# linnanwang/FastGen

Hardware: AMD Instinct MI355X
Metric: images/sec at 4-step distilled (DMD2) sampling (higher is better)
Workload: dtype fp32 (tensors, accumulate) with split-bf16 x3 MFMA conv products; 1 GPU; EDM CIFAR-10 32x32 SongUNet (55.7M params) DMD2 4-step 'sde' sampling, batch=512 per GPU; global_batch=512, sample_steps=4, parallelism=replicas x1 (no data-path collective), graph=True

## Files before the change

### fastgen_amd/csrc/conv_ws3.hip

```cpp
#include "common.h"
#include "conv.h"

namespace {

constexpr int X3_NTHR = 768;
constexpr int X3_KC = 32;
constexpr int X3_PA = 16;
constexpr int X3_PLANE = 3072;
constexpr int X3_ABUF = 8 * X3_PLANE;
constexpr int X3_RING = 4;
constexpr int X3_HOFF = 128 * 512;
constexpr int X3_LDS = X3_HOFF + X3_RING * X3_ABUF;
constexpr int X3_TAPB = 2048;

template <int LOGW>
struct X3Geom {
    static constexpr int W = 1 << LOGW;
    static constexpr int TW = 16, TH = 8;
    static constexpr int IPT = LOGW == 3 ? 2 : 1;
    static constexpr int TCOLS = LOGW == 3 ? 1 : W / TW;
    static constexpr int TPI = LOGW == 3 ? 1 : (W / TH) * TCOLS;
    static constexpr int HW_ = LOGW == 3 ? 2 * W + 3 : TW + 2, HH_ = TH + 2;
    static constexpr int HALO_PIX = HW_ * HH_;
    static constexpr int RS = HW_ * X3_PA;
    static_assert(HALO_PIX * X3_PA <= X3_PLANE && HALO_PIX <= 192, "one halo plane; three producer passes of 64 pixels");
};

__device__ __forceinline__ void x3_barrier() {
    asm volatile("s_waitcnt lgkmcnt(0)\n\ts_barrier" ::: "memory");
}

struct X3Frag {
    bf16x8 hi, lo;
};

template <int RES, int LOGW, int PRO>
__global__ __launch_bounds__(X3_NTHR) void conv3_x3ws_kernel(const ConvArgs a, const int ntiles) {
    using G = X3Geom<LOGW>;
    constexpr bool SUB = RES == RES_SUBPIX;
    constexpr int NTAP = SUB ? 4 : 9;
    constexpr int RN = SUB ? 4 : 3;
    constexpr int NQ = 4 * NTAP;
    constexpr int X3_STEPB = NTAP * X3_TAPB;
    extern __shared__ __attribute__((aligned(16))) char smem[];
    char* const hbuf = smem;
    char* const ring = smem + X3_HOFF;

    const int tid = threadIdx.x;
    const int lane = tid & 63;
    const int wave = __builtin_amdgcn_readfirstlane(tid >> 6);
    const int Cin = a.C1 + a.C2;
    const int nchunk = Cin / X3_KC;
    const int G8 = (int)gridDim.x >> 3;
    const int wg = ((gridDim.x & 7) == 0) ? ((int)blockIdx.x & 7) * G8 + ((int)blockIdx.x >> 3) : (int)blockIdx.x;
    const int gstride = (int)gridDim.x;
    const int my_tiles = (ntiles - wg + gstride - 1) / gstride;
    const int S = my_tiles * nchunk;
    const int NSTEP = S + 3;
    const int H = SUB ? a.Hs : a.H;

    if (wave < 8) {
        const int grp = wave >> 2, wl = wave & 3;
        const int col = lane & 15, g4 = lane >> 4;
        const size_t wstride = (size_t)nchunk * NTAP * 1024;
        const __amdgpu_buffer_rsrc_t wrs = __builtin_amdgcn_make_buffer_rsrc(
            const_cast<__bf16*>(reinterpret_cast<const __bf16*>(a.wpack_ws) + (size_t)(grp * 8 + wl * 2) * wstride), 0, 0x7fffffff,
            0x00020000);
        const int wvoff = lane * 16;
        const int wsb = (int)(wstride * 2);
        const int wphb = SUB ? 16 * wsb : 0;
        int tcur = wg;
        auto load_w = [&](int byte_off) -> X3Frag {
            X3Frag f;
            f.hi = __builtin_bit_cast(bf16x8, __builtin_amdgcn_raw_buffer_load_b128(wrs, wvoff, byte_off, 0));
            f.lo = __builtin_bit_cast(bf16x8, __builtin_amdgcn_raw_buffer_load_b128(wrs, wvoff, byte_off + 1024, 0));
            return f;
        };
        X3Frag wq[RN][2];
#pragma unroll
        for (int j = 0; j < RN; ++j)
#pragma unroll
            for (int nt = 0; nt < 2; ++nt) wq[j][nt] = load_w((tcur & 3) * wphb + nt * wsb + j * X3_TAPB);

        f32x4 acc[8][2];
#pragma unroll
        for (int m = 0; m < 8; ++m)
#pragma unroll
            for (int nt = 0; nt < 2; ++nt) acc[m][nt] = f32x4{0.f, 0.f, 0.f, 0.f};

        const int lane_off = g4 * X3_PLANE + (col + ((G::IPT == 2 && col >= 8) ? 1 : 0)) * X3_PA;
        const int dl0 = col * 512 + ((8 * wl + ((g4) ^ (col & 7))) << 4);
        const int dl1 = col * 512 + ((8 * wl + ((4 + g4) ^ (col & 7))) << 4);

        x3_barrier();
        int c = 0;
        for (int s = 0; s < NSTEP; ++s) {
            const int ls = s - 2 * grp;
            if (ls >= 0 && ls < S) {
                const char* abase = ring + (ls & 3) * X3_ABUF + lane_off + (SUB ? ((tcur >> 1) & 1) * G::RS + (tcur & 1) * X3_PA : 0);
                const int cn = (c + 1 == nchunk) ? 0 : c + 1;
                const int tnext = cn == 0 ? tcur + gstride : tcur;
                const int wcur = (tcur & 3) * wphb + c * X3_STEPB;
                const int wnxt = (ls + 1 < S) ? (tnext & 3) * wphb + cn * X3_STEPB : wcur;
                auto read_x = [&](int q, X3Frag (&xf)[2]) {
                    const int tap = q >> 2, m0 = 2 * (q & 3);
                    const int off = ((SUB ? tap >> 1 : tap / 3) + m0) * G::RS + (SUB ? tap & 1 : tap % 3) * X3_PA;
#pragma unroll
                    for (int m = 0; m < 2; ++m) {
                        xf[m].hi = *reinterpret_cast<const bf16x8*>(abase + off + m * G::RS);
                        xf[m].lo = *reinterpret_cast<const bf16x8*>(abase + off + m * G::RS + 4 * X3_PLANE);
                    }
                };
                auto mma12 = [&](int q, const X3Frag (&xf)[2]) {
                    const int tap = q >> 2, m0 = 2 * (q & 3);
                    const X3Frag(&wf)[2] = wq[tap % RN];
#pragma unroll
                    for (int m = 0; m < 2; ++m)
#pragma unroll
                        for (int nt = 0; nt < 2; ++nt)
                            acc[m0 + m][nt] = __builtin_amdgcn_mfma_f32_16x16x32_bf16(wf[nt].hi, xf[m].lo, acc[m0 + m][nt], 0, 0, 0);
#pragma unroll
                    for (int m = 0; m < 2; ++m)
#pragma unroll
                        for (int nt = 0; nt < 2; ++nt)
                            acc[m0 + m][nt] = __builtin_amdgcn_mfma_f32_16x16x32_bf16(wf[nt].lo, xf[m].hi, acc[m0 + m][nt], 0, 0, 0);
#pragma unroll
                    for (int m = 0; m < 2; ++m)
#pragma unroll
                        for (int nt = 0; nt < 2; ++nt)
                            acc[m0 + m][nt] = __builtin_amdgcn_mfma_f32_16x16x32_bf16(wf[nt].hi, xf[m].hi, acc[m0 + m][nt], 0, 0, 0);
                    if ((q & 3) != 3) return;
                    const int pn = (tap + RN < NTAP) ? wcur + (tap + RN) * X3_TAPB : wnxt + (tap + RN - NTAP) * X3_TAPB;
#pragma unroll
                    for (int nt = 0; nt < 2; ++nt) wq[tap % RN][nt] = load_w(pn + nt * wsb);
                };
                X3Frag x0[2], x1[2];
                read_x(0, x0);
#pragma unroll
                for (int q = 0; q < NQ; q += 2) {
                    read_x(q + 1, x1);
                    __builtin_amdgcn_sched_barrier(0);
                    mma12(q, x0);
                    __builtin_amdgcn_sched_barrier(0);
                    if (q + 2 < NQ) read_x(q + 2, x0);
                    __builtin_amdgcn_sched_barrier(0);
                    mma12(q + 1, x1);
                    __builtin_amdgcn_sched_barrier(0);
                }
                if (c + 1 == nchunk) {
#pragma unroll
                    for (int m = 0; m < 8; ++m) {
                        *reinterpret_cast<f32x4*>(hbuf + m * 8192 + dl0) = acc[m][0];
                        *reinterpret_cast<f32x4*>(hbuf + m * 8192 + dl1) = acc[m][1];
                        acc[m][0] = f32x4{0.f, 0.f, 0.f, 0.f};
                        acc[m][1] = f32x4{0.f, 0.f, 0.f, 0.f};
                    }
                }
                c = cn;
                tcur = tnext;
            }
            x3_barrier();
        }
        return;
    }

    const int ptid = tid - 512;
    const int pw = wave - 8;
    const int oct = ptid & 3;
    const float* src1 = reinterpret_cast<const float*>(a.src1);
    const float* src2 = reinterpret_cast<const float*>(a.src2);
    int hdy[3], hdx[3], hlds[3];
    bool third;
    const int pslot = ptid >> 2;
    const int pimg = (G::IPT == 2 && pslot >= 30) ? 1 : 0;
#pragma unroll
    for (int i = 0; i < 3; ++i) {
        int hy, hx;
        if (G::IPT == 2) {
            const int l = pimg ? min(pslot - 30 + 34 * i, 99) : pslot + 30 * i;
            hy = pimg ? l / 10 : l / 9;
            hx = pimg ? 9 + (l - hy * 10) : l - hy * 9;
            third = pimg ? pslot - 30 + 68 < 100 : true;
        } else {
            const int hq = min(pslot + 64 * i, G::HALO_PIX - 1);
            hy = hq / G::HW_;
            hx = hq - hy * G::HW_;
            third = pslot + 128 < G::HALO_PIX;
        }
        hdy[i] = hy - 1;
        hdx[i] = hx - 1 - pimg * (G::W + 1);
        hlds[i] = oct * X3_PLANE + hy * G::RS + hx * X3_PA;
    }

    auto tile_coord = [&](int t, int& n, int& slot, int& row0, int& col0) {
        if (SUB) t >>= 2;
        n = t * G::IPT / G::TPI;
        slot = t - n * G::TPI / G::IPT;
        row0 = (slot / G::TCOLS) * G::TH;
        col0 = (slot % G::TCOLS) * G::TW;
    };

    struct Staged {
        f32x4 raw[3][2];
        float2 ab[8];
    };
    unsigned off1[3], off2[3];
    bool valid[3];
    const float2* abn = a.ab;
    auto tile_setup = [&](int t) __attribute__((always_inline)) {
        int n, slot, row0, col0;
        tile_coord(t, n, slot, row0, col0);
        bool in_batch = true;
        if (G::IPT == 2) {
            n += pimg;
            in_batch = n < a.B;
            n = min(n, a.B - 1);
        }
#pragma unroll
        for (int i = 0; i < 3; ++i) {
            const int y = row0 + hdy[i], x = col0 + hdx[i];
            valid[i] = (y >= 0) && (y < H) && (x >= 0) && (x < G::W) && (i < 2 || third) && in_batch;
            const int yc = min(max(y, 0), H - 1), xc = min(max(x, 0), G::W - 1);
            const int sy = (RES == RES_UP) ? (yc >> 1) : yc, sx = (RES == RES_UP) ? (xc >> 1) : xc;
            const unsigned pix = (unsigned)((n * a.Hs + sy) * a.Ws + sx);
            off1[i] = (pix * (unsigned)a.C1 + oct * 8) * 4u;
            off2[i] = (pix * (unsigned)a.C2 + oct * 8) * 4u;
        }
        abn = a.ab + (size_t)n * Cin;
    };
    auto stage_load = [&](Staged& st, int t, int c32) __attribute__((always_inline)) {
        if (c32 == 0) tile_setup(t);
        const bool first = c32 * X3_KC < a.C1;
        const char* base = first ? reinterpret_cast<const char*>(src1) + c32 * (X3_KC * 4)
                                 : reinterpret_cast<const char*>(src2) + (c32 * X3_KC - a.C1) * 4;
#pragma unroll
        for (int i = 0; i < 3; ++i) {
            const char* p = base + (first ? off1[i] : off2[i]);
            st.raw[i][0] = *reinterpret_cast<const f32x4*>(p);
            st.raw[i][1] = *reinterpret_cast<const f32x4*>(p + 16);
        }
        if (PRO == PRO_NONE) return;
        const float2* p = abn + c32 * X3_KC + oct * 8;
#pragma unroll
        for (int j = 0; j < 8; j += 2) {
            const f32x4 q = *reinterpret_cast<const f32x4*>(p + j);
            st.ab[j] = make_float2(q[0], q[1]);
            st.ab[j + 1] = make_float2(q[2], q[3]);
        }
    };
    auto stage_store = [&](const Staged& st, char* abuf) __attribute__((always_inline)) {
#pragma unroll
        for (int i = 0; i < 3; ++i) {
            float v[8];
#pragma unroll
            for (int j = 0; j < 8; ++j) {
                v[j] = st.raw[i][j >> 2][j & 3];
                if (PRO != PRO_NONE) v[j] = silu_f<true>(fmaf(v[j], st.ab[j].x, st.ab[j].y));
            }
            bf16x8 hi, lo;
            split8(v, hi, lo);
            typedef __attribute__((ext_vector_type(4))) unsigned u32x4;
            u32x4 wh = __builtin_bit_cast(u32x4, hi), wl_ = __builtin_bit_cast(u32x4, lo);
#pragma unroll
            for (int j = 0; j < 4; ++j) {
                wh[j] = valid[i] ? wh[j] : 0u;
                wl_[j] = valid[i] ? wl_[j] : 0u;
            }
            if (i < 2 || third) {
                *reinterpret_cast<u32x4*>(abuf + hlds[i]) = wh;
                *reinterpret_cast<u32x4*>(abuf + hlds[i] + 4 * X3_PLANE) = wl_;
            }
        }
    };

    const int chq = lane & 31, psub = lane >> 5;
    float* const out = reinterpret_cast<float*>(a.out);
    const float* const resid = reinterpret_cast<const float*>(a.resid);
    const bool has_resid = __builtin_amdgcn_readfirstlane(resid != nullptr);
    auto retire_half = [&](int t, int half) __attribute__((always_inline)) {
        int n, slot, row0, col0;
        tile_coord(t, n, slot, row0, col0);
        const int co = half * 128 + chq * 4;
        const int nimg = G::IPT == 2 ? min(2, a.B - n) : 1;
        f32x4 radd[G::IPT];
#pragma unroll
        for (int k = 0; k < G::IPT; ++k) {
            radd[k] = f32x4{0.f, 0.f, 0.f, 0.f};
            if (a.bias) radd[k] = *reinterpret_cast<const f32x4*>(a.bias + co);
            const int nk = G::IPT == 2 ? min(n + k, a.B - 1) : n;
            if (a.temb) radd[k] += *reinterpret_cast<const f32x4*>(a.temb + (size_t)nk * a.temb_stride + co);
            radd[k] *= a.scale;
        }
        constexpr int OW = SUB ? 2 * G::W : G::W, OST = SUB ? 2 : 1;
        const int ph = t & 3;
        const size_t tb = SUB ? (((size_t)n * (2 * H) + 2 * row0 + (ph >> 1)) * OW + 2 * col0 + (ph & 1)) * 256 + co
                              : (((size_t)n * H + row0) * G::W + col0) * 256 + co;
        const int rs = (SUB || G::IPT == 2) ? 0 : a.rshift;
        const size_t rtb = (SUB || G::IPT == 2) ? tb : (((size_t)n * (H >> rs) + (row0 >> rs)) * (G::W >> rs) + (col0 >> rs)) * 256 + co;
        float ssum[G::IPT] = {}, ssq[G::IPT] = {};
#pragma unroll 1
        for (int grp8 = 0; grp8 < 2; ++grp8) {
            f32x4 rr[8], dv[8];
            unsigned go[8];
#pragma unroll
            for (int j = 0; j < 8; ++j) {
                const int px = pw * 32 + 2 * (grp8 * 8 + j) + psub;
                unsigned rgo;
                if (G::IPT == 2) {
                    go[j] = (unsigned)((((j >> 2) * OW + OST * (px >> 4)) * OW + OST * (px & 7)) * 256);
                    rgo = go[j];
                } else {
                    go[j] = (unsigned)((OST * (px >> 4) * OW + OST * (px & 15)) * 256);
                    rgo = SUB ? go[j] : (unsigned)((((px >> 4) >> rs) * (G::W >> rs) + ((px & 15) >> rs)) * 256);
                }
                rr[j] = f32x4{0.f, 0.f, 0.f, 0.f};
                if (has_resid && (G::IPT == 1 || (j >> 2) < nimg)) rr[j] = *reinterpret_cast<const f32x4*>(resid + rtb + rgo);
                dv[j] = *reinterpret_cast<const f32x4*>(hbuf + px * 512 + ((chq ^ (px & 7)) << 4));
            }
#pragma unroll
            for (int j = 0; j < 8; ++j) {
                const int k = G::IPT == 2 ? j >> 2 : 0;
                if (G::IPT == 2 && k >= nimg) continue;
                f32x4 v;
#pragma unroll
                for (int e = 0; e < 4; ++e) v[e] = fmaf(dv[j][e], a.scale, radd[k][e]);
                if (has_resid) {
#pragma unroll
                    for (int e = 0; e < 4; ++e) v[e] = fmaf(rr[j][e], a.scale, v[e]);
                }
                *reinterpret_cast<f32x4*>(out + tb + go[j]) = v;
                ssum[k] += (v[0] + v[1]) + (v[2] + v[3]);
                ssq[k] += (v[0] * v[0] + v[1] * v[1]) + (v[2] * v[2] + v[3] * v[3]);
            }
        }
#pragma unroll
        for (int k = 0; k < G::IPT; ++k) {
            ssum[k] += __shfl_xor(ssum[k], 32);
            ssq[k] += __shfl_xor(ssq[k], 32);
            const size_t sl = SUB ? ((size_t)(n + k) * G::TPI + slot) * 4 + ph : (size_t)(n + k) * G::TPI + slot;
            if (a.stats && psub == 0 && k < nimg) a.stats[(sl * 4 + pw) * 64 + half * 32 + chq] = make_float2(ssum[k], ssq[k]);
        }
    };

    auto advance = [&](int& t, int& cc) {
        if (++cc == nchunk) {
            cc = 0;
            t += gstride;
        }
    };
    Staged st;
    int t1 = wg, c1 = 0;
    stage_load(st, t1, c1);
    stage_store(st, ring);
    advance(t1, c1);
    x3_barrier();
    int sa = 0;
    for (int s = 0; s < NSTEP; ++s) {
        const bool more = s + 1 < S;
        if (more) stage_load(st, t1, c1);
        if (sa == 0 && s >= nchunk && s <= S) retire_half(wg + (s / nchunk - 1) * gstride, 0);
        if (sa == 2 % nchunk && s - 2 >= nchunk && s - 2 <= S && (s - 2) % nchunk == 0) retire_half(wg + ((s - 2) / nchunk - 1) * gstride, 1);
        if (more) {
            stage_store(st, ring + ((s + 1) & 3) * X3_ABUF);
            advance(t1, c1);
        }
        if (++sa == nchunk) sa = 0;
        x3_barrier();
    }
}

__global__ void pack_conv_weights_x3ws_kernel(const float* __restrict__ w, __bf16* __restrict__ out, int cout, int cin) {
    const size_t total = (size_t)cout * cin * 9;
    const int nstep = cin / X3_KC;
    for (size_t idx = (size_t)blockIdx.x * blockDim.x + threadIdx.x; idx < total; idx += (size_t)gridDim.x * blockDim.x) {
        size_t t = idx;
        const int j = t % 8; t /= 8;
        const int lane = t % 64; t /= 64;
        const int tap = t % 9; t /= 9;
        const int step = t % nstep; t /= nstep;
        const int n16 = (int)t;
        const int co = n16 * 16 + (lane & 15);
        const int ci = step * X3_KC + 8 * (lane >> 4) + j;
        const float v = w[((size_t)co * cin + ci) * 9 + tap];
        const __bf16 hi = (__bf16)v;
        const size_t o = (idx / 512) * 1024 + (idx % 512);
        out[o] = hi;
        out[o + 512] = (__bf16)(v - (float)hi);
    }
}

__global__ void pack_conv_weights_x3sub_kernel(const float* __restrict__ w, __bf16* __restrict__ out, int cout, int cin) {
    const size_t total = (size_t)16 * cout * cin;
    const int nstep = cin / X3_KC, ng = cout / 16;
    for (size_t idx = (size_t)blockIdx.x * blockDim.x + threadIdx.x; idx < total; idx += (size_t)gridDim.x * blockDim.x) {
        size_t t = idx;
        const int j = t % 8; t /= 8;
        const int lane = t % 64; t /= 64;
        const int tap = t % 4; t /= 4;
        const int step = t % nstep; t /= nstep;
        const int n16 = t % ng; t /= ng;
        const int py = (int)t >> 1, px = (int)t & 1, ty = tap >> 1, tx = tap & 1;
        const int co = n16 * 16 + (lane & 15);
        const int ci = step * X3_KC + 8 * (lane >> 4) + j;
        const int ky0 = py ? 2 * ty : ty, ky1 = py ? ty + 1 : 2 * ty;
        const int kx0 = px ? 2 * tx : tx, kx1 = px ? tx + 1 : 2 * tx;
        const float* wp = w + ((size_t)co * cin + ci) * 9;
        float v = 0.f;
        for (int ky = ky0; ky <= ky1; ++ky)
            for (int kx = kx0; kx <= kx1; ++kx) v += wp[ky * 3 + kx];
        const __bf16 hi = (__bf16)v;
        const size_t o = (idx / 512) * 1024 + (idx % 512);
        out[o] = hi;
        out[o + 512] = (__bf16)(v - (float)hi);
    }
}

int g_x3_cus[16] = {};

template <int RES, int LOGW, int PRO>
int launch_x3_one(const ConvArgs& a, hipStream_t stream, bool prepare_only) {
    using G = X3Geom<LOGW>;
    auto kern = conv3_x3ws_kernel<RES, LOGW, PRO>;
    int dev = 0;
    if (hipGetDevice(&dev) != hipSuccess || dev < 0 || dev >= 16) return (int)hipErrorInvalidDevice;
    static bool attr_done[16] = {};
    if (!attr_done[dev]) {
        hipError_t e = hipFuncSetAttribute(reinterpret_cast<const void*>(kern), hipFuncAttributeMaxDynamicSharedMemorySize, X3_LDS);
        if (e != hipSuccess) return (int)e;
        attr_done[dev] = true;
    }
    if (!g_x3_cus[dev]) {
        int n = 0;
        if (hipDeviceGetAttribute(&n, hipDeviceAttributeMultiprocessorCount, dev) != hipSuccess || n <= 0) return (int)hipErrorUnknown;
        g_x3_cus[dev] = n;
    }
    if (prepare_only) return 0;
    const int ntiles = (a.B * G::TPI + G::IPT - 1) / G::IPT * (RES == RES_SUBPIX ? 4 : 1);
    const int grid = ntiles < g_x3_cus[dev] ? ntiles : g_x3_cus[dev];
    hipLaunchKernelGGL(kern, dim3(grid), dim3(X3_NTHR), X3_LDS, stream, a, ntiles);
    return (int)hipGetLastError();
}

}

int conv_x3ws_stat_slots(int W, int res) {
    if (res == RES_SUBPIX) return (W == 32 ? X3Geom<4>::TPI : X3Geom<3>::TPI) * 16;
    return (W == 32 ? X3Geom<5>::TPI : W == 16 ? X3Geom<4>::TPI : X3Geom<3>::TPI) * 4;
}

bool conv_x3ws_shape_ok(int cout, int cin, int res) {
    return cout == 256 && (res == 32 || res == 16 || res == 8) && (cin % X3_KC) == 0 && cin / X3_KC >= 4;
}

bool conv_x3ws_supported(int ks, int pro, int res, int outmode, const ConvArgs& a) {
    const int cin = a.C1 + a.C2;
    const size_t src_bytes = (size_t)a.B * a.Hs * a.Ws * (size_t)(a.C1 > a.C2 ? a.C1 : a.C2) * 4;
    if (src_bytes >= (1ull << 32)) return false;
    if (res == RES_SUBPIX)
        return ks == 3 && outmode == OUT_NHWC && pro == PRO_GN_SILU && a.ab && a.H == a.W && a.Hs == a.Ws && a.H == 2 * a.Hs && (a.Ws == 16 || a.Ws == 8) &&
               conv_x3ws_shape_ok(a.Cout, cin, a.Ws) && (a.C1 % X3_KC) == 0 && a.wpack_ws && !a.rshift;
    if (ks != 3 || outmode != OUT_NHWC || a.H != a.W || !conv_x3ws_shape_ok(a.Cout, cin, a.W) || (a.C1 % X3_KC) || !a.wpack_ws) return false;
    if (a.W == 8 && res != RES_NONE) return false;
    if (a.rshift && (a.rshift != 1 || !a.resid || a.W == 8 || res != RES_NONE)) return false;
    if (pro == PRO_NONE) return res == RES_NONE && a.Hs == a.H && a.Ws == a.W;
    return pro == PRO_GN_SILU && (res == RES_NONE || res == RES_UP) && a.ab != nullptr;
}

int launch_conv_x3ws(int res, const ConvArgs& a, hipStream_t stream, bool prepare_only, int pro) {
    if (res == RES_SUBPIX) {
        if (pro != PRO_GN_SILU || (a.Ws != 16 && a.Ws != 8)) return (int)hipErrorInvalidValue;
        return a.Ws == 16 ? launch_x3_one<RES_SUBPIX, 4, PRO_GN_SILU>(a, stream, prepare_only) : launch_x3_one<RES_SUBPIX, 3, PRO_GN_SILU>(a, stream, prepare_only);
    }
    if (pro == PRO_NONE || a.W == 8) {
        if (res != RES_NONE) return (int)hipErrorInvalidValue;
        if (a.W == 8)
            return pro == PRO_NONE ? launch_x3_one<RES_NONE, 3, PRO_NONE>(a, stream, prepare_only)
                                   : launch_x3_one<RES_NONE, 3, PRO_GN_SILU>(a, stream, prepare_only);
        return a.W == 32 ? launch_x3_one<RES_NONE, 5, PRO_NONE>(a, stream, prepare_only) : launch_x3_one<RES_NONE, 4, PRO_NONE>(a, stream, prepare_only);
    }
    if (a.W == 32)
        return res == RES_UP ? launch_x3_one<RES_UP, 5, PRO_GN_SILU>(a, stream, prepare_only) : launch_x3_one<RES_NONE, 5, PRO_GN_SILU>(a, stream, prepare_only);
    return res == RES_UP ? launch_x3_one<RES_UP, 4, PRO_GN_SILU>(a, stream, prepare_only) : launch_x3_one<RES_NONE, 4, PRO_GN_SILU>(a, stream, prepare_only);
}

int launch_pack_conv_weights_x3ws(const float* w_oihw, void* wpack_ws, int cout, int cin, hipStream_t stream) {
    const size_t total = (size_t)cout * cin * 9;
    const int grid = (int)((total + 255) / 256 < 4096 ? (total + 255) / 256 : 4096);
    hipLaunchKernelGGL(pack_conv_weights_x3ws_kernel, dim3(grid), dim3(256), 0, stream, w_oihw, (__bf16*)wpack_ws, cout, cin);
    return (int)hipGetLastError();
}

int launch_pack_conv_weights_x3sub(const float* w_oihw, void* wpack_sub, int cout, int cin, hipStream_t stream) {
    const size_t total = (size_t)16 * cout * cin;
    const int grid = (int)((total + 255) / 256 < 4096 ? (total + 255) / 256 : 4096);
    hipLaunchKernelGGL(pack_conv_weights_x3sub_kernel, dim3(grid), dim3(256), 0, stream, w_oihw, (__bf16*)wpack_sub, cout, cin);
    return (int)hipGetLastError();
}
```

Before: 2832 img/s.

## Interleave paired 8x8 images in LDS halo and skip zero-padding rows

For the 8x8 resolution where two images share a tile, the halo layout now interleaves the two images column-wise (slot = 2*x + img) with a single shared padding row that wraps. Padding slots are zero-filled once at kernel start instead of being written on every stage. The MFMA loop skips reads and multiplies for rows that are always padding in the non-subpixel case, and the producer needs only two staging passes instead of three. The epilogue assigns one image per lane half, which removes the per-image loops and the cross-lane shuffle. Compile-time checks verify that LDS reads are bank-conflict free and that the slot mapping covers every position, but the change adds considerable indexing complexity.

```diff
diff --git a/fastgen_amd/csrc/conv_ws3.hip b/fastgen_amd/csrc/conv_ws3.hip
--- a/fastgen_amd/csrc/conv_ws3.hip
+++ b/fastgen_amd/csrc/conv_ws3.hip
@@ -20,11 +20,71 @@
     static constexpr int IPT = LOGW == 3 ? 2 : 1;
     static constexpr int TCOLS = LOGW == 3 ? 1 : W / TW;
     static constexpr int TPI = LOGW == 3 ? 1 : (W / TH) * TCOLS;
-    static constexpr int HW_ = LOGW == 3 ? 2 * W + 3 : TW + 2, HH_ = TH + 2;
+    static constexpr int HW_ = IPT == 2 ? 2 * (W + 2) : TW + 2, HH_ = IPT == 2 ? TH + 1 : TH + 2;
     static constexpr int HALO_PIX = HW_ * HH_;
     static constexpr int RS = HW_ * X3_PA;
+    static constexpr int NI = IPT == 2 ? 2 : 3;
+    static constexpr int ZSLOTS = IPT == 2 ? HALO_PIX - 2 * W * W : 0;
     static_assert(HALO_PIX * X3_PA <= X3_PLANE && HALO_PIX <= 192, "one halo plane; three producer passes of 64 pixels");
+
+    static constexpr int prow(int r) { return (IPT == 2 && r == TH + 1) ? 0 : r; }
+    static constexpr int pix_slot(int img, int y, int x) { return prow(y + 1) * HW_ + (IPT == 2 ? 2 * (x + 1) + img : x + 1); }
+    static constexpr int read_slot(int col, int r, int c) { return prow(r) * HW_ + col + IPT * c; }
+    static constexpr int stage_pix(int ps, int i) { return (ps & 31) + 32 * i; }
+    static constexpr int stage_slot(int ps, int i) { return pix_slot(ps >> 5, stage_pix(ps, i) >> 3, stage_pix(ps, i) & 7); }
+    static constexpr int zero_slot(int z) { return z < HW_ ? z : (1 + ((z - HW_) >> 2)) * HW_ + ((z - HW_) & 3) + (((z - HW_) & 2) ? HW_ - 4 : 0); }
+    static constexpr bool is_zero_slot(int s) { return IPT == 2 && (s < HW_ || s % HW_ < 2 || s % HW_ >= HW_ - 2); }
 };
+
+constexpr int x3_b128_group(int lane) {
+    const int l = lane & 31;
+    return 2 * (lane >> 5) + ((l < 4 || (l >= 12 && l < 16) || (l >= 20 && l < 28)) ? 0 : 1);
+}
+template <int LOGW>
+constexpr bool x3_reads_conflict_free() {
+    using G = X3Geom<LOGW>;
+    for (int r = 0; r <= G::TH + 1; ++r)
+        for (int c = 0; c < 3; ++c)
+            for (int grp = 0; grp < 4; ++grp) {
+                unsigned seen = 0;
+                for (int lane = 0; lane < 64; ++lane) {
+                    if (x3_b128_group(lane) != grp) continue;
+                    const int byte = (lane >> 4) * X3_PLANE + G::read_slot(lane & 15, r, c) * X3_PA;
+                    const unsigned bit = 1u << ((byte >> 4) & 15);
+                    if (seen & bit) return false;
+                    seen |= bit;
+                }
+            }
+    return true;
+}
+constexpr bool x3_pair_layout_ok() {
+    using G = X3Geom<3>;
+    for (int col = 0; col < 16; ++col)
+        for (int r = 0; r <= G::TH + 1; ++r)
+            for (int c = 0; c < 3; ++c) {
+                const int img = col & 1, y = r - 1, x = (col >> 1) + c - 1;
+                const int s = G::read_slot(col, r, c);
+                const bool pad = y < 0 || y >= G::W || x < 0 || x >= G::W;
+                if (s != G::pix_slot(img, y, x) || G::is_zero_slot(s) != pad || s < 0 || s >= G::HALO_PIX) return false;
+            }
+    bool used[G::HALO_PIX] = {};
+    for (int ps = 0; ps < 64; ++ps)
+        for (int i = 0; i < G::NI; ++i) {
+            const int p = G::stage_pix(ps, i), s = G::stage_slot(ps, i);
+            if (p < 0 || p >= G::W * G::W || s < 0 || s >= G::HALO_PIX || G::is_zero_slot(s) || used[s]) return false;
+            used[s] = true;
+        }
+    for (int z = 0; z < G::ZSLOTS; ++z) {
+        const int s = G::zero_slot(z);
+        if (s < 0 || s >= G::HALO_PIX || !G::is_zero_slot(s) || used[s]) return false;
+        used[s] = true;
+    }
+    for (int s = 0; s < G::HALO_PIX; ++s)
+        if (!used[s]) return false;
+    return true;
+}
+static_assert(x3_reads_conflict_free<3>() && x3_reads_conflict_free<4>() && x3_reads_conflict_free<5>(), "activation reads: one LDS cycle per lane group");
+static_assert(X3Geom<3>::ZSLOTS == 52 && x3_pair_layout_ok(), "8x8 pair layout: reads, staging and zero fill");
 
 __device__ __forceinline__ void x3_barrier() {
     asm volatile("s_waitcnt lgkmcnt(0)\n\ts_barrier" ::: "memory");
@@ -88,7 +148,7 @@
 #pragma unroll
             for (int nt = 0; nt < 2; ++nt) acc[m][nt] = f32x4{0.f, 0.f, 0.f, 0.f};
 
-        const int lane_off = g4 * X3_PLANE + (col + ((G::IPT == 2 && col >= 8) ? 1 : 0)) * X3_PA;
+        const int lane_off = g4 * X3_PLANE + G::read_slot(col, 0, 0) * X3_PA;
         const int dl0 = col * 512 + ((8 * wl + ((g4) ^ (col & 7))) << 4);
         const int dl1 = col * 512 + ((8 * wl + ((4 + g4) ^ (col & 7))) << 4);
 
@@ -97,18 +157,24 @@
         for (int s = 0; s < NSTEP; ++s) {
             const int ls = s - 2 * grp;
             if (ls >= 0 && ls < S) {
-                const char* abase = ring + (ls & 3) * X3_ABUF + lane_off + (SUB ? ((tcur >> 1) & 1) * G::RS + (tcur & 1) * X3_PA : 0);
+                const int py = SUB ? (tcur >> 1) & 1 : 0, px = SUB ? tcur & 1 : 0;
+                const char* abase = ring + (ls & 3) * X3_ABUF + lane_off + (SUB ? G::read_slot(0, py, px) * X3_PA : 0);
+                const int wrap = (SUB && G::IPT == 2 && py) ? -(G::TH + 1) * G::RS : 0;
                 const int cn = (c + 1 == nchunk) ? 0 : c + 1;
                 const int tnext = cn == 0 ? tcur + gstride : tcur;
                 const int wcur = (tcur & 3) * wphb + c * X3_STEPB;
                 const int wnxt = (ls + 1 < S) ? (tnext & 3) * wphb + cn * X3_STEPB : wcur;
+                auto zero_row = [](int tap, int m) { return !SUB && G::IPT == 2 && (tap / 3 + m == 0 || tap / 3 + m == G::TH + 1); };
                 auto read_x = [&](int q, X3Frag (&xf)[2]) {
                     const int tap = q >> 2, m0 = 2 * (q & 3);
-                    const int off = ((SUB ? tap >> 1 : tap / 3) + m0) * G::RS + (SUB ? tap & 1 : tap % 3) * X3_PA;
+                    const int ty = SUB ? tap >> 1 : tap / 3, tx = SUB ? tap & 1 : tap % 3;
 #pragma unroll
                     for (int m = 0; m < 2; ++m) {
-                        xf[m].hi = *reinterpret_cast<const bf16x8*>(abase + off + m * G::RS);
-                        xf[m].lo = *reinterpret_cast<const bf16x8*>(abase + off + m * G::RS + 4 * X3_PLANE);
+                        if (zero_row(tap, m0 + m)) continue;
+                        const int r = ty + m0 + m;
+                        const int off = G::read_slot(0, r, tx) * X3_PA + ((SUB && G::IPT == 2 && r == G::TH) ? wrap : 0);
+                        xf[m].hi = *reinterpret_cast<const bf16x8*>(abase + off);
+                        xf[m].lo = *reinterpret_cast<const bf16x8*>(abase + off + 4 * X3_PLANE);
                     }
                 };
                 auto mma12 = [&](int q, const X3Frag (&xf)[2]) {
@@ -118,17 +184,20 @@
                     for (int m = 0; m < 2; ++m)
 #pragma unroll
                         for (int nt = 0; nt < 2; ++nt)
-                            acc[m0 + m][nt] = __builtin_amdgcn_mfma_f32_16x16x32_bf16(wf[nt].hi, xf[m].lo, acc[m0 + m][nt], 0, 0, 0);
+                            if (!zero_row(tap, m0 + m))
+                                acc[m0 + m][nt] = __builtin_amdgcn_mfma_f32_16x16x32_bf16(wf[nt].hi, xf[m].lo, acc[m0 + m][nt], 0, 0, 0);
 #pragma unroll
                     for (int m = 0; m < 2; ++m)
 #pragma unroll
                         for (int nt = 0; nt < 2; ++nt)
-                            acc[m0 + m][nt] = __builtin_amdgcn_mfma_f32_16x16x32_bf16(wf[nt].lo, xf[m].hi, acc[m0 + m][nt], 0, 0, 0);
+                            if (!zero_row(tap, m0 + m))
+                                acc[m0 + m][nt] = __builtin_amdgcn_mfma_f32_16x16x32_bf16(wf[nt].lo, xf[m].hi, acc[m0 + m][nt], 0, 0, 0);
 #pragma unroll
                     for (int m = 0; m < 2; ++m)
 #pragma unroll
                         for (int nt = 0; nt < 2; ++nt)
-                            acc[m0 + m][nt] = __builtin_amdgcn_mfma_f32_16x16x32_bf16(wf[nt].hi, xf[m].hi, acc[m0 + m][nt], 0, 0, 0);
+                            if (!zero_row(tap, m0 + m))
+                                acc[m0 + m][nt] = __builtin_amdgcn_mfma_f32_16x16x32_bf16(wf[nt].hi, xf[m].hi, acc[m0 + m][nt], 0, 0, 0);
                     if ((q & 3) != 3) return;
                     const int pn = (tap + RN < NTAP) ? wcur + (tap + RN) * X3_TAPB : wnxt + (tap + RN - NTAP) * X3_TAPB;
 #pragma unroll
@@ -169,27 +238,33 @@
     const int oct = ptid & 3;
     const float* src1 = reinterpret_cast<const float*>(a.src1);
     const float* src2 = reinterpret_cast<const float*>(a.src2);
-    int hdy[3], hdx[3], hlds[3];
-    bool third;
+    constexpr int NI = G::NI;
+    int hdy[NI], hdx[NI], hlds[NI];
+    bool third = true;
     const int pslot = ptid >> 2;
-    const int pimg = (G::IPT == 2 && pslot >= 30) ? 1 : 0;
-#pragma unroll
-    for (int i = 0; i < 3; ++i) {
-        int hy, hx;
+    const int pimg = G::IPT == 2 ? pslot >> 5 : 0;
+#pragma unroll
+    for (int i = 0; i < NI; ++i) {
         if (G::IPT == 2) {
-            const int l = pimg ? min(pslot - 30 + 34 * i, 99) : pslot + 30 * i;
-            hy = pimg ? l / 10 : l / 9;
-            hx = pimg ? 9 + (l - hy * 10) : l - hy * 9;
-            third = pimg ? pslot - 30 + 68 < 100 : true;
+            const int p = G::stage_pix(pslot, i);
+            hdy[i] = p >> 3;
+            hdx[i] = p & 7;
+            hlds[i] = oct * X3_PLANE + G::stage_slot(pslot, i) * X3_PA;
         } else {
             const int hq = min(pslot + 64 * i, G::HALO_PIX - 1);
-            hy = hq / G::HW_;
-            hx = hq - hy * G::HW_;
+            const int hy = hq / G::HW_, hx = hq - hy * G::HW_;
             third = pslot + 128 < G::HALO_PIX;
-        }
-        hdy[i] = hy - 1;
-        hdx[i] = hx - 1 - pimg * (G::W + 1);
-        hlds[i] = oct * X3_PLANE + hy * G::RS + hx * X3_PA;
+            hdy[i] = hy - 1;
+            hdx[i] = hx - 1;
+            hlds[i] = oct * X3_PLANE + hy * G::RS + hx * X3_PA;
+        }
+    }
+    if constexpr (G::IPT == 2) {
+        typedef __attribute__((ext_vector_type(4))) unsigned u32x4;
+        for (int idx = ptid; idx < X3_RING * 8 * G::ZSLOTS; idx += 256) {
+            const int plane = idx / G::ZSLOTS;
+            *reinterpret_cast<u32x4*>(ring + plane * X3_PLANE + G::zero_slot(idx - plane * G::ZSLOTS) * X3_PA) = u32x4{0u, 0u, 0u, 0u};
+        }
     }
 
     auto tile_coord = [&](int t, int& n, int& slot, int& row0, int& col0) {
@@ -201,11 +276,11 @@
     };
 
     struct Staged {
-        f32x4 raw[3][2];
+        f32x4 raw[NI][2];
         float2 ab[8];
     };
-    unsigned off1[3], off2[3];
-    bool valid[3];
+    unsigned off1[NI], off2[NI];
+    bool valid[NI];
     const float2* abn = a.ab;
     auto tile_setup = [&](int t) __attribute__((always_inline)) {
         int n, slot, row0, col0;
@@ -217,10 +292,10 @@
             n = min(n, a.B - 1);
         }
 #pragma unroll
-        for (int i = 0; i < 3; ++i) {
+        for (int i = 0; i < NI; ++i) {
             const int y = row0 + hdy[i], x = col0 + hdx[i];
-            valid[i] = (y >= 0) && (y < H) && (x >= 0) && (x < G::W) && (i < 2 || third) && in_batch;
-            const int yc = min(max(y, 0), H - 1), xc = min(max(x, 0), G::W - 1);
+            valid[i] = G::IPT == 2 ? in_batch : (y >= 0) && (y < H) && (x >= 0) && (x < G::W) && (i < 2 || third);
+            const int yc = G::IPT == 2 ? y : min(max(y, 0), H - 1), xc = G::IPT == 2 ? x : min(max(x, 0), G::W - 1);
             const int sy = (RES == RES_UP) ? (yc >> 1) : yc, sx = (RES == RES_UP) ? (xc >> 1) : xc;
             const unsigned pix = (unsigned)((n * a.Hs + sy) * a.Ws + sx);
             off1[i] = (pix * (unsigned)a.C1 + oct * 8) * 4u;
@@ -234,7 +309,7 @@
         const char* base = first ? reinterpret_cast<const char*>(src1) + c32 * (X3_KC * 4)
                                  : reinterpret_cast<const char*>(src2) + (c32 * X3_KC - a.C1) * 4;
 #pragma unroll
-        for (int i = 0; i < 3; ++i) {
+        for (int i = 0; i < NI; ++i) {
             const char* p = base + (first ? off1[i] : off2[i]);
             st.raw[i][0] = *reinterpret_cast<const f32x4*>(p);
             st.raw[i][1] = *reinterpret_cast<const f32x4*>(p + 16);
@@ -249,8 +324,17 @@
         }
     };
     auto stage_store = [&](const Staged& st, char* abuf) __attribute__((always_inline)) {
-#pragma unroll
-        for (int i = 0; i < 3; ++i) {
+        typedef __attribute__((ext_vector_type(4))) unsigned u32x4;
+        if (G::IPT == 2 && !__builtin_amdgcn_readfirstlane((int)valid[0])) {
+#pragma unroll
+            for (int i = 0; i < NI; ++i) {
+                *reinterpret_cast<u32x4*>(abuf + hlds[i]) = u32x4{0u, 0u, 0u, 0u};
+                *reinterpret_cast<u32x4*>(abuf + hlds[i] + 4 * X3_PLANE) = u32x4{0u, 0u, 0u, 0u};
+            }
+            return;
+        }
+#pragma unroll
+        for (int i = 0; i < NI; ++i) {
             float v[8];
 #pragma unroll
             for (int j = 0; j < 8; ++j) {
@@ -259,12 +343,13 @@
             }
             bf16x8 hi, lo;
             split8(v, hi, lo);
-            typedef __attribute__((ext_vector_type(4))) unsigned u32x4;
             u32x4 wh = __builtin_bit_cast(u32x4, hi), wl_ = __builtin_bit_cast(u32x4, lo);
-#pragma unroll
-            for (int j = 0; j < 4; ++j) {
-                wh[j] = valid[i] ? wh[j] : 0u;
-                wl_[j] = valid[i] ? wl_[j] : 0u;
+            if (G::IPT == 1) {
+#pragma unroll
+                for (int j = 0; j < 4; ++j) {
+                    wh[j] = valid[i] ? wh[j] : 0u;
+                    wl_[j] = valid[i] ? wl_[j] : 0u;
+                }
             }
             if (i < 2 || third) {
                 *reinterpret_cast<u32x4*>(abuf + hlds[i]) = wh;
@@ -281,23 +366,20 @@
         int n, slot, row0, col0;
         tile_coord(t, n, slot, row0, col0);
         const int co = half * 128 + chq * 4;
-        const int nimg = G::IPT == 2 ? min(2, a.B - n) : 1;
-        f32x4 radd[G::IPT];
-#pragma unroll
-        for (int k = 0; k < G::IPT; ++k) {
-            radd[k] = f32x4{0.f, 0.f, 0.f, 0.f};
-            if (a.bias) radd[k] = *reinterpret_cast<const f32x4*>(a.bias + co);
-            const int nk = G::IPT == 2 ? min(n + k, a.B - 1) : n;
-            if (a.temb) radd[k] += *reinterpret_cast<const f32x4*>(a.temb + (size_t)nk * a.temb_stride + co);
-            radd[k] *= a.scale;
-        }
+        const int img = G::IPT == 2 ? psub : 0;
+        const bool live = G::IPT == 1 || n + img < a.B;
+        f32x4 radd = f32x4{0.f, 0.f, 0.f, 0.f};
+        if (a.bias) radd = *reinterpret_cast<const f32x4*>(a.bias + co);
+        const int nk = G::IPT == 2 ? min(n + img, a.B - 1) : n;
+        if (a.temb) radd += *reinterpret_cast<const f32x4*>(a.temb + (size_t)nk * a.temb_stride + co);
+        radd *= a.scale;
         constexpr int OW = SUB ? 2 * G::W : G::W, OST = SUB ? 2 : 1;
         const int ph = t & 3;
         const size_t tb = SUB ? (((size_t)n * (2 * H) + 2 * row0 + (ph >> 1)) * OW + 2 * col0 + (ph & 1)) * 256 + co
                               : (((size_t)n * H + row0) * G::W + col0) * 256 + co;
         const int rs = (SUB || G::IPT == 2) ? 0 : a.rshift;
         const size_t rtb = (SUB || G::IPT == 2) ? tb : (((size_t)n * (H >> rs) + (row0 >> rs)) * (G::W >> rs) + (col0 >> rs)) * 256 + co;
-        float ssum[G::IPT] = {}, ssq[G::IPT] = {};
+        float ssum = 0.f, ssq = 0.f;
 #pragma unroll 1
         for (int grp8 = 0; grp8 < 2; ++grp8) {
             f32x4 rr[8], dv[8];
@@ -307,39 +389,37 @@
                 const int px = pw * 32 + 2 * (grp8 * 8 + j) + psub;
                 unsigned rgo;
                 if (G::IPT == 2) {
-                    go[j] = (unsigned)((((j >> 2) * OW + OST * (px >> 4)) * OW + OST * (px & 7)) * 256);
+                    go[j] = (unsigned)((((img * OW + OST * (px >> 4)) * OW + OST * ((px & 15) >> 1)) * 256));
                     rgo = go[j];
                 } else {
                     go[j] = (unsigned)((OST * (px >> 4) * OW + OST * (px & 15)) * 256);
                     rgo = SUB ? go[j] : (unsigned)((((px >> 4) >> rs) * (G::W >> rs) + ((px & 15) >> rs)) * 256);
                 }
                 rr[j] = f32x4{0.f, 0.f, 0.f, 0.f};
-                if (has_resid && (G::IPT == 1 || (j >> 2) < nimg)) rr[j] = *reinterpret_cast<const f32x4*>(resid + rtb + rgo);
+                if (has_resid && live) rr[j] = *reinterpret_cast<const f32x4*>(resid + rtb + rgo);
                 dv[j] = *reinterpret_cast<const f32x4*>(hbuf + px * 512 + ((chq ^ (px & 7)) << 4));
             }
+            if (!live) continue;
 #pragma unroll
             for (int j = 0; j < 8; ++j) {
-                const int k = G::IPT == 2 ? j >> 2 : 0;
-                if (G::IPT == 2 && k >= nimg) continue;
                 f32x4 v;
 #pragma unroll
-                for (int e = 0; e < 4; ++e) v[e] = fmaf(dv[j][e], a.scale, radd[k][e]);
+                for (int e = 0; e < 4; ++e) v[e] = fmaf(dv[j][e], a.scale, radd[e]);
                 if (has_resid) {
 #pragma unroll
                     for (int e = 0; e < 4; ++e) v[e] = fmaf(rr[j][e], a.scale, v[e]);
                 }
                 *reinterpret_cast<f32x4*>(out + tb + go[j]) = v;
-                ssum[k] += (v[0] + v[1]) + (v[2] + v[3]);
-                ssq[k] += (v[0] * v[0] + v[1] * v[1]) + (v[2] * v[2] + v[3] * v[3]);
-            }
-        }
-#pragma unroll
-        for (int k = 0; k < G::IPT; ++k) {
-            ssum[k] += __shfl_xor(ssum[k], 32);
-            ssq[k] += __shfl_xor(ssq[k], 32);
-            const size_t sl = SUB ? ((size_t)(n + k) * G::TPI + slot) * 4 + ph : (size_t)(n + k) * G::TPI + slot;
-            if (a.stats && psub == 0 && k < nimg) a.stats[(sl * 4 + pw) * 64 + half * 32 + chq] = make_float2(ssum[k], ssq[k]);
-        }
+                ssum += (v[0] + v[1]) + (v[2] + v[3]);
+                ssq += (v[0] * v[0] + v[1] * v[1]) + (v[2] * v[2] + v[3] * v[3]);
+            }
+        }
+        if (G::IPT == 1) {
+            ssum += __shfl_xor(ssum, 32);
+            ssq += __shfl_xor(ssq, 32);
+        }
+        const size_t sl = SUB ? ((size_t)(n + img) * G::TPI + slot) * 4 + ph : (size_t)(n + img) * G::TPI + slot;
+        if (a.stats && live && (G::IPT == 2 || psub == 0)) a.stats[(sl * 4 + pw) * 64 + half * 32 + chq] = make_float2(ssum, ssq);
     };
 
     auto advance = [&](int& t, int& cc) {
```

Result: no change. 2847 img/s, median of 6 (+0.5%).

## Reorder non-SUB 3x3 conv loop by input row to reuse LDS fragments and skip padded halo rows

Applied to the files above, without the earlier changes.

For the non-subsampled 3x3 path, the inner loop now iterates over halo input rows (column tap x row) instead of over taps. Each LDS fragment is read once and applied to up to three output rows, which cuts LDS reads for the activation operand. MFMAs on the zero-padded top and bottom halo rows are skipped at image edges. The weight register ring now holds one column-tap per kernel row and is refilled when the last output row of that row-tap finishes, which changes the prefetch order and may shift register pressure and scheduling.

```diff
diff --git a/fastgen_amd/csrc/conv_ws3.hip b/fastgen_amd/csrc/conv_ws3.hip
--- a/fastgen_amd/csrc/conv_ws3.hip
+++ b/fastgen_amd/csrc/conv_ws3.hip
@@ -80,7 +80,7 @@
 #pragma unroll
         for (int j = 0; j < RN; ++j)
 #pragma unroll
-            for (int nt = 0; nt < 2; ++nt) wq[j][nt] = load_w((tcur & 3) * wphb + nt * wsb + j * X3_TAPB);
+            for (int nt = 0; nt < 2; ++nt) wq[j][nt] = load_w((tcur & 3) * wphb + nt * wsb + (SUB ? j : 3 * j) * X3_TAPB);
 
         f32x4 acc[8][2];
 #pragma unroll
@@ -102,50 +102,92 @@
                 const int tnext = cn == 0 ? tcur + gstride : tcur;
                 const int wcur = (tcur & 3) * wphb + c * X3_STEPB;
                 const int wnxt = (ls + 1 < S) ? (tnext & 3) * wphb + cn * X3_STEPB : wcur;
-                auto read_x = [&](int q, X3Frag (&xf)[2]) {
-                    const int tap = q >> 2, m0 = 2 * (q & 3);
-                    const int off = ((SUB ? tap >> 1 : tap / 3) + m0) * G::RS + (SUB ? tap & 1 : tap % 3) * X3_PA;
-#pragma unroll
-                    for (int m = 0; m < 2; ++m) {
-                        xf[m].hi = *reinterpret_cast<const bf16x8*>(abase + off + m * G::RS);
-                        xf[m].lo = *reinterpret_cast<const bf16x8*>(abase + off + m * G::RS + 4 * X3_PLANE);
+                if constexpr (!SUB) {
+                    const int trow = (tcur % G::TPI) / G::TCOLS;
+                    const bool top = G::IPT == 2 || trow == 0;
+                    const bool bot = G::IPT == 2 || trow == G::W / G::TH - 1;
+                    auto read_row = [&](int i, X3Frag& xf) {
+                        const int tx = i / G::HH_, h = i % G::HH_;
+                        if ((h == 0 && top) || (h == G::HH_ - 1 && bot)) return;
+                        xf.hi = *reinterpret_cast<const bf16x8*>(abase + h * G::RS + tx * X3_PA);
+                        xf.lo = *reinterpret_cast<const bf16x8*>(abase + h * G::RS + tx * X3_PA + 4 * X3_PLANE);
+                    };
+                    auto mma_row = [&](int i, const X3Frag& xf) {
+                        const int tx = i / G::HH_, h = i % G::HH_;
+                        const bool live = !((h == 0 && top) || (h == G::HH_ - 1 && bot));
+#pragma unroll
+                        for (int ty = 0; ty < 3; ++ty) {
+                            const int m = h - ty;
+                            if (m < 0 || m >= G::TH) continue;
+                            if (live) {
+#pragma unroll
+                                for (int term = 0; term < 3; ++term)
+#pragma unroll
+                                    for (int nt = 0; nt < 2; ++nt)
+                                        acc[m][nt] = __builtin_amdgcn_mfma_f32_16x16x32_bf16(term == 1 ? wq[ty][nt].lo : wq[ty][nt].hi,
+                                                                                             term == 0 ? xf.lo : xf.hi, acc[m][nt], 0, 0, 0);
+                            }
+                            if (m != G::TH - 1) continue;
+                            const int pn = (tx < 2 ? wcur + (3 * ty + tx + 1) * X3_TAPB : wnxt + 3 * ty * X3_TAPB);
+#pragma unroll
+                            for (int nt = 0; nt < 2; ++nt) wq[ty][nt] = load_w(pn + nt * wsb);
+                        }
+                    };
+                    X3Frag xr[2];
+                    read_row(0, xr[0]);
+#pragma unroll
+                    for (int i = 0; i < 3 * G::HH_; ++i) {
+                        if (i + 1 < 3 * G::HH_) read_row(i + 1, xr[(i + 1) & 1]);
+                        __builtin_amdgcn_sched_barrier(0);
+                        mma_row(i, xr[i & 1]);
+                        __builtin_amdgcn_sched_barrier(0);
                     }
-                };
-                auto mma12 = [&](int q, const X3Frag (&xf)[2]) {
-                    const int tap = q >> 2, m0 = 2 * (q & 3);
-                    const X3Frag(&wf)[2] = wq[tap % RN];
-#pragma unroll
-                    for (int m = 0; m < 2; ++m)
-#pragma unroll
-                        for (int nt = 0; nt < 2; ++nt)
-                            acc[m0 + m][nt] = __builtin_amdgcn_mfma_f32_16x16x32_bf16(wf[nt].hi, xf[m].lo, acc[m0 + m][nt], 0, 0, 0);
-#pragma unroll
-                    for (int m = 0; m < 2; ++m)
-#pragma unroll
-                        for (int nt = 0; nt < 2; ++nt)
-                            acc[m0 + m][nt] = __builtin_amdgcn_mfma_f32_16x16x32_bf16(wf[nt].lo, xf[m].hi, acc[m0 + m][nt], 0, 0, 0);
-#pragma unroll
-                    for (int m = 0; m < 2; ++m)
-#pragma unroll
-                        for (int nt = 0; nt < 2; ++nt)
-                            acc[m0 + m][nt] = __builtin_amdgcn_mfma_f32_16x16x32_bf16(wf[nt].hi, xf[m].hi, acc[m0 + m][nt], 0, 0, 0);
-                    if ((q & 3) != 3) return;
-                    const int pn = (tap + RN < NTAP) ? wcur + (tap + RN) * X3_TAPB : wnxt + (tap + RN - NTAP) * X3_TAPB;
-#pragma unroll
-                    for (int nt = 0; nt < 2; ++nt) wq[tap % RN][nt] = load_w(pn + nt * wsb);
-                };
-                X3Frag x0[2], x1[2];
-                read_x(0, x0);
-#pragma unroll
-                for (int q = 0; q < NQ; q += 2) {
-                    read_x(q + 1, x1);
-                    __builtin_amdgcn_sched_barrier(0);
-                    mma12(q, x0);
-                    __builtin_amdgcn_sched_barrier(0);
-                    if (q + 2 < NQ) read_x(q + 2, x0);
-                    __builtin_amdgcn_sched_barrier(0);
-                    mma12(q + 1, x1);
-                    __builtin_amdgcn_sched_barrier(0);
+                } else {
+                    auto read_x = [&](int q, X3Frag (&xf)[2]) {
+                        const int tap = q >> 2, m0 = 2 * (q & 3);
+                        const int off = ((tap >> 1) + m0) * G::RS + (tap & 1) * X3_PA;
+#pragma unroll
+                        for (int m = 0; m < 2; ++m) {
+                            xf[m].hi = *reinterpret_cast<const bf16x8*>(abase + off + m * G::RS);
+                            xf[m].lo = *reinterpret_cast<const bf16x8*>(abase + off + m * G::RS + 4 * X3_PLANE);
+                        }
+                    };
+                    auto mma12 = [&](int q, const X3Frag (&xf)[2]) {
+                        const int tap = q >> 2, m0 = 2 * (q & 3);
+                        const X3Frag(&wf)[2] = wq[tap % RN];
+#pragma unroll
+                        for (int m = 0; m < 2; ++m)
+#pragma unroll
+                            for (int nt = 0; nt < 2; ++nt)
+                                acc[m0 + m][nt] = __builtin_amdgcn_mfma_f32_16x16x32_bf16(wf[nt].hi, xf[m].lo, acc[m0 + m][nt], 0, 0, 0);
+#pragma unroll
+                        for (int m = 0; m < 2; ++m)
+#pragma unroll
+                            for (int nt = 0; nt < 2; ++nt)
+                                acc[m0 + m][nt] = __builtin_amdgcn_mfma_f32_16x16x32_bf16(wf[nt].lo, xf[m].hi, acc[m0 + m][nt], 0, 0, 0);
+#pragma unroll
+                        for (int m = 0; m < 2; ++m)
+#pragma unroll
+                            for (int nt = 0; nt < 2; ++nt)
+                                acc[m0 + m][nt] = __builtin_amdgcn_mfma_f32_16x16x32_bf16(wf[nt].hi, xf[m].hi, acc[m0 + m][nt], 0, 0, 0);
+                        if ((q & 3) != 3) return;
+                        const int pn = (tap + RN < NTAP) ? wcur + (tap + RN) * X3_TAPB : wnxt + (tap + RN - NTAP) * X3_TAPB;
+#pragma unroll
+                        for (int nt = 0; nt < 2; ++nt) wq[tap % RN][nt] = load_w(pn + nt * wsb);
+                    };
+                    X3Frag x0[2], x1[2];
+                    read_x(0, x0);
+#pragma unroll
+                    for (int q = 0; q < NQ; q += 2) {
+                        read_x(q + 1, x1);
+                        __builtin_amdgcn_sched_barrier(0);
+                        mma12(q, x0);
+                        __builtin_amdgcn_sched_barrier(0);
+                        if (q + 2 < NQ) read_x(q + 2, x0);
+                        __builtin_amdgcn_sched_barrier(0);
+                        mma12(q + 1, x1);
+                        __builtin_amdgcn_sched_barrier(0);
+                    }
                 }
                 if (c + 1 == nchunk) {
 #pragma unroll
```

New measurement: 2865 img/s before, 2916 img/s after, median of 6. 1.02x the previous value.
